# FindoraNetwork/ark-bulletproofs

Measured on AMD Instinct MI355X. Metric: r1cs_constraints_proved_per_sec (+ r1cs_batch_verifies_per_sec under "verify"), higher is better.
Workload: dtype u32x9 (256-bit modular integers, radix 2^29)

## Files before the change

### ark_bulletproofs_amd/csrc/arkbp.hip

```cpp
#include <hip/hip_runtime.h>
#include <sys/prctl.h>
#include <time.h>
#include <rccl/rccl.h>
#include <dlfcn.h>
#include <mutex>
#include <cmath>
#include <cstdio>
#include <cstring>
#include <algorithm>
#include <deque>
#include <array>
#include <functional>
#include <map>
#include <memory>
#include <set>
#include <string>
#include <tuple>
#include <unordered_map>
#include <vector>
#include "../../include/arkbp.h"
#include <atomic>
#include <chrono>
#include "host_proto.hpp"
#include "prove_steps.hpp"
// ... 780 lines not shown
    HIPCHK(ctx_stream_wait(ctx));
    HIPCHK(hipGetLastError());
    const double t_m3 = mtrace ? tnow() : 0;
    result = use_marginals ? msm_horner_tail<C>((const u64*)ctx->h_T, pl.W * pl.c, 0, 0, 1) : msm_horner_tail<C>((const u64*)ctx->h_T, 0, pl.W, nblk_ws, pl.c);
    if (mtrace) fprintf(stderr, "[msm] n=%zu c=%d W=%d K=%d  front(enqueue+sync) %.1f us  back enqueue %.1f us  back wait %.1f us  host tail %.1f us\n", n, pl.c, pl.W, K,
                        (t_m1 - t_m0) * 1e6, (t_m2 - t_m1) * 1e6, (t_m3 - t_m2) * 1e6, (tnow() - t_m3) * 1e6);
    return finish_sharded(result);
}

struct FbRun { int table; size_t first, count; size_t stride = 1; };
template <class C> static int fb_rows_build(hipStream_t st, const u32* gens, u32* table, size_t count, size_t table_cap, size_t slab, DevBuf& tmp, DevBuf& pref, DevBuf& outb) {
    for (size_t lo = 0; lo < count; lo += slab) {
        const size_t m = std::min(slab, count - lo);
        const u32 gb = (u32)((m + 255) / 256);
        hipLaunchKernelGGL(k_msm_fb_rows<C>, dim3(gb), dim3(256), 0, st, gens + lo * 16, tmp.as<u32>(), (u32)m, FB_ROWS);
        hipLaunchKernelGGL(k_ftab_normalize<C>, dim3(gb), dim3(256), 0, st, tmp.as<u32>(), pref.as<u32>(), outb.as<u32>(), (u32)m, FB_ROWS);
        HIPCHK(hipGetLastError());
        for (u32 r = 0; r < FB_ROWS; r++)
            HIPCHK(hipMemcpyAsync(table + ((size_t)r * table_cap + lo) * 16, outb.as<u32>() + (size_t)r * m * 16, m * 64, hipMemcpyDeviceToDevice, st));
    }
    return BP_OK;
}
template <class C> static int fb_tables_build(bp_ctx* ctx, size_t cap) {
    hipStream_t st = ctx->stream;
    if (cap == 0 || cap > ctx->gens_cap) { g_err = "msm tables: more bases than installed generators"; return BP_E_GENS_LENGTH; }
    if (!ctx->d_G.owned) { g_err = "msm tables: build them on the ctx that owns the generator tables, then bp_gens_share"; return BP_E_ARG; }
    ctx->fb_cap = 0;
    BPCHK(ctx->fb_G.ensure_exact((size_t)FB_ROWS * cap * 64)); BPCHK(ctx->fb_H.ensure_exact((size_t)FB_ROWS * cap * 64)); BPCHK(ctx->fb_pc.ensure((size_t)FB_ROWS * 2 * 64));
    const size_t slab = std::min<size_t>(cap, (size_t)1 << 18);
    DevBuf tmp, pref, outb;
    BPCHK(tmp.ensure(FB_ROWS * slab * 96)); BPCHK(pref.ensure(FB_ROWS * slab * 32)); BPCHK(outb.ensure(FB_ROWS * slab * 64));
// ... 360 lines not shown
    typedef host::Fld<typename C::Fr> S;
    memset(&d, 0, sizeof d);
    d.nwin = (u32)ctx->ftab_nwin;
    if (d.nwin > 44) return false;
    if constexpr (C::HAS_GLV) {
        GlvRaw raw; u32 dummy[5];
        if (!glv_decompose<C>(t, dummy, dummy, dummy, dummy, &raw)) return false;
        ftab_recode(raw.mg1, 3, raw.n1, ctx->ftab_w, ctx->ftab_nwin, d.e1, d.neg1);
        ftab_recode(raw.mg2, 3, raw.n2, ctx->ftab_w, ctx->ftab_nwin, d.e2, d.neg2);
    } else {
        uint64_t c[4]; S::to_canon(c, t);
        ftab_recode(c, 4, false, ctx->ftab_w, ctx->ftab_nwin, d.e1, d.neg1);
    }
    return true;
}
template <class C> static int ftab_build(bp_ctx* ctx, size_t n, int w, size_t budget_bytes, u32 first = 0, u32 stride = 1) {
    hipStream_t st = ctx->stream;
    if (n == 0 || stride == 0 || (size_t)first + (n - 1) * (size_t)stride >= ctx->gens_cap) { g_err = "fold tables: more bases than installed generators"; return BP_E_GENS_LENGTH; }
    if (!ctx->d_G.owned && stride == 1) { g_err = "fold tables: build them on the ctx that owns the generator tables, then bp_gens_share"; return BP_E_ARG; }
    for (DevBuf* b : {&ctx->ftab_G, &ctx->ftab_H}) { if (!b->owned) { b->p = nullptr; b->cap = 0; b->owned = true; } else b->release(); }
    ctx->ftab_n = 0; ctx->ftab_first = 0; ctx->ftab_stride = 1;
    size_t free_b = 0, total_b = 0;
    HIPCHK(hipMemGetInfo(&free_b, &total_b));
    if (!budget_bytes) budget_bytes = free_b / 4 * 3;
    auto bytes_for = [&](int ww) { const size_t E = (size_t)1 << (ww - 1); return 2 * (size_t)ftab_nwin_for<C>(ww) * E * n * 64 + E * n * (96 + 32) + n * 96; };
    if (w == 0) { w = 8; while (w > 2 && bytes_for(w) > budget_bytes) w--; }
    if (w < 2 || w > 8 || bytes_for(w) > free_b) { g_err = "fold tables: not enough device memory"; return BP_E_ARG; }
    const size_t E = (size_t)1 << (w - 1);
    const int nwin = ftab_nwin_for<C>(w);
    const size_t per_vec = (size_t)nwin * E * n * 64;
    BPCHK(ctx->ftab_G.ensure_exact(per_vec)); BPCHK(ctx->ftab_H.ensure_exact(per_vec));
    DevBuf tmp, pref, state, gsl;
    BPCHK(tmp.ensure_exact(E * n * 96)); BPCHK(pref.ensure_exact(E * n * 32)); BPCHK(state.ensure_exact(n * 96));
    const u32 gb = (u32)((n + 255) / 256);
    if (stride > 1 || first) BPCHK(gsl.ensure_exact(n * 64));
    for (int v = 0; v < 2; v++) {
        const u32* gens = v ? ctx->d_H.as<u32>() : ctx->d_G.as<u32>();
        if (gsl.p) {
            hipLaunchKernelGGL(k_cyclic_gather<Blk64>, dim3(gb), dim3(256), 0, st, gens, gsl.as<u32>(), (u32)n, first, stride);
            gens = gsl.as<u32>();
        }
        u32* T = v ? ctx->ftab_H.as<u32>() : ctx->ftab_G.as<u32>();
        for (int j = 0; j < nwin; j++) {
            hipLaunchKernelGGL(k_ftab_window<C>, dim3(gb), dim3(256), 0, st, gens, state.as<u32>(), tmp.as<u32>(), (u32)n, (u32)E, j == 0 ? 1 : 0);
            hipLaunchKernelGGL(k_ftab_normalize<C>, dim3(gb), dim3(256), 0, st, tmp.as<u32>(), pref.as<u32>(), T + (size_t)j * E * n * 16, (u32)n, (u32)E);
        }
    }
    HIPCHK(hipGetLastError());
    HIPCHK(ctx_stream_wait(ctx));
    tmp.release(); pref.release(); state.release(); gsl.release();
    ctx->ftab_n = n; ctx->ftab_w = w; ctx->ftab_nwin = nwin; ctx->ftab_first = first; ctx->ftab_stride = stride;
    return BP_OK;
}
template <class C> static int tables_check(bp_ctx* ctx, uint64_t* bad_fold, uint64_t* bad_rows) {
    hipStream_t st = ctx->stream;
    BPCHK(ctx->io_out.ensure(64));
    unsigned long long* d_bad = ctx->io_out.as<unsigned long long>();
    HIPCHK(hipMemsetAsync(d_bad, 0, 16, st));
    if (ctx->ftab_n) {
        const u32 n = (u32)ctx->ftab_n, E = 1u << (ctx->ftab_w - 1), gb = (n + 255) / 256;
// ... 137 lines not shown
    IpaState s;
    if (!ladder) {
        if (!ctx->ftab_n || !ctx->ftab_G.p || !ctx->ftab_H.p) { g_err = "bp_debug_fold: the fold tables are not built (bp_gens_fold_tables)"; return BP_E_ARG; }
        if (!stride || (size_t)first + (in_pts - 1) * (size_t)stride >= ctx->gens_cap) { g_err = "bp_debug_fold: an element lies outside the installed generators"; return BP_E_ARG; }
        s.gens_first = first; s.gens_stride = stride;
        u32 c0 = 0, cs = 1;
        const size_t tabled = tab2 ? 3 * n : n;
        if (!ftab_cols(ctx, s, c0, cs) || (size_t)c0 + (tabled - 1) * (size_t)cs >= ctx->ftab_n) { g_err = "bp_debug_fold: an element lies outside the fold tables"; return BP_E_ARG; }
    }
    DevBuf wG, wH, out;
    auto done = [&](int rc) { wG.release(); wH.release(); out.release(); return rc; };
#define DFCHK(x) do { int rc__ = (x); if (rc__ != BP_OK) return done(rc__); } while (0)
#define DFHIP(x) do { if ((x) != hipSuccess) { g_err = "bp_debug_fold: HIP error"; return done(BP_E_HIP); } } while (0)
    DFCHK(wG.ensure_exact(in_pts * 64)); DFCHK(wH.ensure_exact(in_pts * 64)); DFCHK(out.ensure_exact(2 * n * 64));
    u32 *d_G = wG.as<u32>(), *d_H = wH.as<u32>();
    if (ladder) {
        DFHIP(hipMemcpyAsync(d_G, G_xy, 2 * n * 64, hipMemcpyHostToDevice, st));
        DFHIP(hipMemcpyAsync(d_H, H_xy, 2 * n * 64, hipMemcpyHostToDevice, st));
        DFCHK(bp_points_import(ctx, d_G, d_G, 2 * n)); DFCHK(bp_points_import(ctx, d_H, d_H, 2 * n));
    } else if (whole) {
        s.d_G_in = ctx->d_G.as<u32>(); s.d_H_in = ctx->d_H.as<u32>();
    } else {
        const u32 gb = (u32)((in_pts + 255) / 256);
        hipLaunchKernelGGL(k_cyclic_gather<Blk64>, dim3(gb), dim3(256), 0, st, ctx->d_G.as<u32>(), d_G, (u32)in_pts, first, stride);
        hipLaunchKernelGGL(k_cyclic_gather<Blk64>, dim3(gb), dim3(256), 0, st, ctx->d_H.as<u32>(), d_H, (u32)in_pts, first, stride);
        s.d_G_in = d_G; s.d_H_in = d_H;
    }
    ctx->fold_took = 0;
    bool ran = true;
    if (ladder) DFCHK(launch_uniform_fold<C>(ctx, d_G, d_H, n, tG, tH, 3, route == BP_DEBUG_FOLD_LADDER_NAF));
    else if (!tab2) DFCHK(launch_tab_fold<C>(ctx, s, d_G, d_H, n, tG, tH, ran));
    else { s.def_tG = tG; s.def_tH = tH; DFCHK(launch_tab_fold2<C>(ctx, s, d_G, d_H, n, t2G, t2H, ran)); }
    DFHIP(hipGetLastError());
    *took = ran ? ctx->fold_took : 0;
    if (ran) {
        DFCHK(bp_points_export(ctx, d_G, out.p, n)); DFCHK(bp_points_export(ctx, d_H, out.as<u32>() + n * 16, n));
        DFHIP(hipMemcpyAsync(G_out, out.p, n * 64, hipMemcpyDeviceToHost, st));
        DFHIP(hipMemcpyAsync(H_out, out.as<u32>() + n * 16, n * 64, hipMemcpyDeviceToHost, st));
    }
    DFHIP(ctx_stream_wait(ctx));
#undef DFCHK
#undef DFHIP
    return done(BP_OK);
}

static inline u32 dt_base_pc(int which ) { return (u32)which; }
static inline u32 dt_base_G(const bp_ctx* ctx, size_t i) { (void)ctx; return (u32)(2 + i); }
static inline u32 dt_base_H(const bp_ctx* ctx, size_t i) { return (u32)(2 + ctx->dt_cap + i); }
template <class C> static int dt_ensure(bp_ctx* ctx, size_t N, bool& ready) {
    ready = false;
    if (!ctx->tune_direct_max || N == 0 || N > ctx->tune_direct_max || ctx->shard_world > 1 || ctx->gens_cap < N) return BP_OK;
    if (ctx->dt_cap >= N) { ready = true; return BP_OK; }
    if (!ctx->dt_tab.owned && ctx->dt_tab.p) { ctx->dt_tab.p = nullptr; ctx->dt_tab.cap = 0; ctx->dt_tab.owned = true; }
// ... 2095 lines not shown
        const bool built = t.p && size && t.cap >= size;
        *dptr = built ? t.p : nullptr; *nbytes = built ? size : 0;
        return BP_OK;
    }
    DevBuf& b = which == 0 ? c->ftab_G : which == 1 ? c->ftab_H : which == 2 ? c->fb_G : c->fb_H;
    const size_t used = which < 2 ? (c->ftab_n ? (size_t)c->ftab_nwin * ((size_t)1 << (c->ftab_w - 1)) * c->ftab_n * 64 : 0) : (size_t)FB_ROWS * c->fb_cap * 64;
    *dptr = used ? b.p : nullptr; *nbytes = used;
    return BP_OK;
}
int bp_debug_fold(bp_ctx* c, int route, size_t n, const uint64_t tG[4], const uint64_t tH[4], const uint64_t t2G[4], const uint64_t t2H[4], uint32_t gens_first,
                  uint32_t gens_stride, const uint64_t* G_xy, const uint64_t* H_xy, uint64_t* G_out_xy, uint64_t* H_out_xy, uint32_t* took) {
    if (!c || route < BP_DEBUG_FOLD_LADDER || route > BP_DEBUG_FOLD_TAB2 || !n || n >= ((size_t)1 << 28) || !tG || !tH || !G_out_xy || !H_out_xy || !took) {
        g_err = "bp_debug_fold: bad argument"; return BP_E_ARG;
    }
    if (route == BP_DEBUG_FOLD_TAB2 && (!t2G || !t2H)) { g_err = "bp_debug_fold: the second multipliers are missing"; return BP_E_ARG; }
    if (route <= BP_DEBUG_FOLD_LADDER_NAF && (!G_xy || !H_xy)) { g_err = "bp_debug_fold: the ladder routes fold the caller's points"; return BP_E_ARG; }
    if (c->host_only) return BP_E_NO_DEVICE;
    HIPCHK(hipSetDevice(c->device));
    return c->curve == 0 ? dbg_fold<Secq>(c, route, n, tG, tH, t2G, t2H, gens_first, gens_stride, G_xy, H_xy, G_out_xy, H_out_xy, took)
                         : dbg_fold<Zorro>(c, route, n, tG, tH, t2G, t2H, gens_first, gens_stride, G_xy, H_xy, G_out_xy, H_out_xy, took);
}
int bp_debug_msm_direct(bp_ctx* c, size_t njobs, const uint32_t* desc, const uint64_t* imm, const uint64_t* const* scalars, const size_t* scalar_lens,
                        uint64_t* out_xy, uint32_t* workgroups) {
    if (!c || !desc || !out_xy || njobs < 1 || njobs > (size_t)DT_MAXOUT) { g_err = "bp_debug_msm_direct: bad argument"; return BP_E_ARG; }
    if (c->host_only) return BP_E_NO_DEVICE;
    if (!c->dt_cap || !c->dt_tab.p) { g_err = "bp_debug_msm_direct: the direct tables are not built (bp_gens_direct_tables)"; return BP_E_ARG; }
    HIPCHK(hipSetDevice(c->device));
    return c->curve == 0 ? dbg_msm_direct<Secq>(c, njobs, desc, imm, scalars, scalar_lens, out_xy, workgroups)
                         : dbg_msm_direct<Zorro>(c, njobs, desc, imm, scalars, scalar_lens, out_xy, workgroups);
}
int bp_gens_download(bp_ctx* c, uint64_t* G_xy, uint64_t* H_xy, size_t n) {
// ... 817 lines not shown
```

### ark_bulletproofs_amd/csrc/ipa.cuh

```cuda
#pragma once
#include "msm.cuh"

namespace arkbp {

template <class F> __global__ void k_scalars_import(const u32* __restrict__ in, u32* __restrict__ out, u32 n) {
    const u32 i = blockIdx.x * blockDim.x + threadIdx.x;
    if (i >= n) return;
    u32 w[8];
    load_words8(w, in + (size_t)i * 8);
    store_fe_dev<F>(out + (size_t)i * 8, fe_load_ark<F>(w));
}
template <class F> __global__ void k_scalars_export(const u32* __restrict__ in, u32* __restrict__ out, u32 n) {
    const u32 i = blockIdx.x * blockDim.x + threadIdx.x;
    if (i >= n) return;
    u32 w[8];
    fe_store_ark<F>(w, load_fe_dev<F>(in + (size_t)i * 8));
    store_words8(out + (size_t)i * 8, w);
}

static constexpr int IMPORT_MAX = 5;
struct ImportList {
    u32* dst[IMPORT_MAX];
    u32 cnt[IMPORT_MAX];
    int nseg;
// ... 298 lines not shown
    if (first) {
        c1 = fe_mul<F>(c1, load_fe_dev<F>(Vf + (size_t)i * 8));
        c2 = fe_mul<F>(c2, load_fe_dev<F>(Vf + (size_t)(n + i) * 8));
    }
    u32 s1[8], s2[8];
    fe_store_canon<F>(s1, c1);
    fe_store_canon<F>(s2, c2);
    const Aff P1 = load_aff_dev(V + (size_t)i * 16), P2 = load_aff_dev(V + (size_t)(n + i) * 16);
    const Jac r = shamir2<C>(P1, P2, s1, s2);
    fold_emit<C>(V, i, t, r, jac_ws);
}

struct Naf {
    u32 plus[9], minus[9];
};
template <class C> __device__ __forceinline__ Jac ladder_madd(const Jac& acc, const Aff& T) {
    bool rare;
    Jac nxt = jac_madd_fast<C>(acc, T, rare);
    if (__builtin_expect(rare, 0)) nxt = jac_madd<C>(acc, T);
    return nxt;
}
template <class C, bool QUAD = false> __global__ void __launch_bounds__(256) __attribute__((amdgpu_waves_per_eu(2)))
k_ipa_fold_uniform(u32* __restrict__ G, u32* __restrict__ H, u32 n, Naf tG, Naf tH, int which ,
                   u32* __restrict__ jac_ws) {
    const u32 tl = blockIdx.x * blockDim.x + threadIdx.x;
    const u32 t = QUAD ? tl >> 2 : tl, ql = threadIdx.x & 3u;
    if (t >= (which == 3 ? 2 * n : n)) return;
    const bool isH = which == 2 || (which == 3 && t >= n);
    const u32 i = (which == 3 && isH) ? t - n : t;
    u32* V = isH ? H : G;
    const Aff P1 = load_aff_dev(V + (size_t)i * 16), P2 = load_aff_dev(V + (size_t)(n + i) * 16);
    const Aff N1 = aff_cneg_lazy<C>(P1, true);
    Jac acc = jac_inf<C>();
#pragma unroll 1
    for (int wd = 8; wd >= 0; wd--) {
        const u32 ep = isH ? tH.plus[wd] : tG.plus[wd], em = isH ? tH.minus[wd] : tG.minus[wd];
#pragma unroll 1
        for (int bit = (wd == 8 ? 0 : 31); bit >= 0; bit--) {
            acc = QUAD ? qjac_dbl<C>(acc, ql) : jac_dbl<C>(acc);
            if (((ep | em) >> bit) & 1) {
                Aff T1 = P1; T1.y = ((em >> bit) & 1) ? N1.y : P1.y;
                acc = QUAD ? qjac_madd<C>(acc, T1, ql) : ladder_madd<C>(acc, T1);
            }
        }
    }
    acc = QUAD ? qjac_madd<C>(acc, P2, ql) : jac_madd<C>(acc, P2);
    if (!QUAD || ql == 0) fold_emit<C>(V, i, t, acc, jac_ws);
}

struct Naf2 {
    u32 p1[5], m1[5], p2[5], m2[5];
};
template <class C, bool QUAD = false> __global__ void __launch_bounds__(256) __attribute__((amdgpu_waves_per_eu(2)))
k_ipa_fold_glv(u32* __restrict__ G, u32* __restrict__ H, u32 n, Naf2 tG, Naf2 tH, int which ,
               u32* __restrict__ jac_ws) {
    typedef typename C::Fq F;
    const u32 tl = blockIdx.x * blockDim.x + threadIdx.x;
    const u32 t = QUAD ? tl >> 2 : tl, ql = threadIdx.x & 3u;
    if (t >= (which == 3 ? 2 * n : n)) return;
    const bool isH = which == 2 || (which == 3 && t >= n);
    const u32 i = (which == 3 && isH) ? t - n : t;
    u32* V = isH ? H : G;
    const Aff P1 = load_aff_dev(V + (size_t)i * 16), P2 = load_aff_dev(V + (size_t)(n + i) * 16);
    Aff Q1;
    Q1.x = fe_canon<F>(fe_mul<F>(P1.x, fe_const<F, C::BETA29>()));
    Q1.y = P1.y;
    const Aff N1 = aff_cneg_lazy<C>(P1, true);
    Jac acc = jac_inf<C>();
#pragma unroll 1
    for (int wd = 4; wd >= 0; wd--) {
        const u32 a = isH ? tH.p1[wd] : tG.p1[wd], b = isH ? tH.m1[wd] : tG.m1[wd];
        const u32 c = isH ? tH.p2[wd] : tG.p2[wd], d = isH ? tH.m2[wd] : tG.m2[wd];
#pragma unroll 1
        for (int bit = (wd == 4 ? 1 : 31); bit >= 0; bit--) {
            acc = QUAD ? qjac_dbl<C>(acc, ql) : jac_dbl<C>(acc);
            if (QUAD) {
                if (((a | b) >> bit) & 1) { Aff T1 = P1; T1.y = ((b >> bit) & 1) ? N1.y : P1.y; acc = qjac_madd<C>(acc, T1, ql); }
                if (((c | d) >> bit) & 1) { Aff T2 = Q1; T2.y = ((d >> bit) & 1) ? N1.y : P1.y; acc = qjac_madd<C>(acc, T2, ql); }
            } else {
#pragma unroll 1
                for (int h = 0; h < 2; h++) {
                    const u32 nz = h ? (c | d) : (a | b), ng = h ? d : b;
                    if ((nz >> bit) & 1) {
                        Aff T;
#pragma unroll
                        for (int l = 0; l < 9; l++) { T.x.l[l] = h ? Q1.x.l[l] : P1.x.l[l]; T.y.l[l] = ((ng >> bit) & 1) ? N1.y.l[l] : P1.y.l[l]; }
                        acc = ladder_madd<C>(acc, T);
                    }
                }
            }
        }
    }
    acc = QUAD ? qjac_madd<C>(acc, P2, ql) : jac_madd<C>(acc, P2);
    if (!QUAD || ql == 0) fold_emit<C>(V, i, t, acc, jac_ws);
}

struct FtabDigits {
    unsigned short e1[44], e2[44];
    unsigned long long neg1, neg2;
    u32 nwin;
};
template <class C> __global__ void __launch_bounds__(256)
k_ftab_window(const u32* __restrict__ gens, u32* __restrict__ state, u32* __restrict__ tmp, u32 n, u32 E, int first) {
    const u32 i = blockIdx.x * blockDim.x + threadIdx.x;
    if (i >= n) return;
    Jac B;
    if (first) { const Aff p = load_aff_dev(gens + (size_t)i * 16); B = jac_madd<C>(jac_inf<C>(), p); }
    else B = load_jac_ws(state + (size_t)i * 24);
    Jac acc = B;
    store_jac_ws<C>(tmp + (size_t)i * 24, acc);
#pragma unroll 1
    for (u32 e = 2; e <= E; e++) {
        acc = jac_add<C>(acc, B);
        store_jac_ws<C>(tmp + ((size_t)(e - 1) * n + i) * 24, acc);
    }
    store_jac_ws<C>(state + (size_t)i * 24, jac_dbl<C>(acc));
}
template <class C> __global__ void __launch_bounds__(256)
k_ftab_normalize(const u32* __restrict__ tmp, u32* __restrict__ pref, u32* __restrict__ out, u32 n, u32 E) {
    typedef typename C::Fq F;
    const u32 i = blockIdx.x * blockDim.x + threadIdx.x;
    if (i >= n) return;
    Fe acc = fe_one<F>();
#pragma unroll 1
    for (u32 e = 0; e < E; e++) {
        u32 w[8];
        load_words8(w, tmp + ((size_t)e * n + i) * 24 + 16);
        const Fe z = fe_unpack(w);
        if (!fe_is_zero_exact(z)) acc = fe_mul<F>(acc, z);
        fe_pack(w, fe_canon<F>(acc));
        store_words8(pref + ((size_t)e * n + i) * 8, w);
    }
    Fe inv = fe_inv<F>(acc);
#pragma unroll 1
    for (int e = (int)E - 1; e >= 0; e--) {
        const Jac P = load_jac_ws(tmp + ((size_t)e * n + i) * 24);
        Aff o;
        if (jac_is_inf(P)) { o.x = fe_zero<F>(); o.y = fe_zero<F>(); }
        else {
            Fe prev = fe_one<F>();
            if (e > 0) { u32 w[8]; load_words8(w, pref + ((size_t)(e - 1) * n + i) * 8); prev = fe_unpack(w); }
            const Fe zinv = fe_mul<F>(inv, prev);
            inv = fe_mul<F>(inv, P.Z);
            o = jac_to_aff_with_zinv<C>(P, zinv);
        }
        u32 w[16];
        aff_store_dev(w, o);
        store_words8(out + ((size_t)e * n + i) * 16, w);
        store_words8(out + ((size_t)e * n + i) * 16 + 8, w + 8);
    }
}
template <class C> __device__ __forceinline__ bool jac_equals_aff(const Jac& J, const Aff& A) {
    typedef typename C::Fq F;
    const bool ji = jac_is_inf(J), ai = aff_is_inf(A);
    if (ji || ai) return ji && ai;
    const Fe zz = fe_sqr<F>(J.Z);
    if (!fe_eq_mod<F>(fe_wred<F>(J.X), fe_mul<F>(A.x, zz))) return false;
    return fe_eq_mod<F>(fe_wred<F>(J.Y), fe_mul<F>(A.y, fe_mul<F>(zz, J.Z)));
}
template <class C> __device__ __forceinline__ bool chain_entry_ok(const u32* __restrict__ cur, const u32* __restrict__ p, const u32* __restrict__ q, bool identity_ok) {
    typedef typename C::Fq F;
    bool canon, unused;
    const Aff A = load_aff_checked<C>(cur, canon);
    const Aff P = load_aff_checked<C>(p, unused);
// ... 123 lines not shown
```

### ark_bulletproofs_amd/csrc/msm.cuh

```cuda
#pragma once
#include "ec.cuh"
#include "fe_io.cuh"
#include "ecq.cuh"
#include "glv.cuh"
#include "msm_plan.hpp"

namespace arkbp {

static constexpr int MSM_MAXSEG = 6;

struct BaseSegs {
    const u32* ptr[MSM_MAXSEG];
    u32 start[MSM_MAXSEG + 1];
    int nseg;
    u32 fixed_c4;
    u32 tbits;
    u64 row_words[MSM_MAXSEG];
    u32 glv;
    u32 stride[MSM_MAXSEG];
};
__device__ __forceinline__ const u32* seg_base_ptr(const BaseSegs& s, u32 idx) {
    u32 w = 0;
    if (s.glv) idx >>= 1;
    if (s.fixed_c4) { w = idx >> s.tbits; idx &= (1u << s.tbits) - 1u; }
    const u32* ptr = s.ptr[0];
    u32 start = s.start[0], sd = s.stride[0];
    u64 rw = s.row_words[0];
#pragma unroll
    for (int j = 1; j < MSM_MAXSEG; j++) {
        const bool in = j < s.nseg && idx >= s.start[j];
        ptr = in ? s.ptr[j] : ptr; start = in ? s.start[j] : start; sd = in ? s.stride[j] : sd; rw = in ? s.row_words[j] : rw;
    }
    sd = sd ? sd : 1u;
    return ptr + (size_t)(idx - start) * sd * 16 + (size_t)(w * s.fixed_c4) * rw;
}

struct ScalSegs {
    const u32* ptr[MSM_MAXSEG];
    u32 start[MSM_MAXSEG + 1];
    int nseg;
};
__device__ __forceinline__ const u32* seg_scalar_ptr(const ScalSegs& s, u32 idx) {
    int k = 0;
#pragma unroll
    for (int j = 1; j < MSM_MAXSEG; j++) k += (j < s.nseg && idx >= s.start[j]) ? 1 : 0;
    return s.ptr[k] + (size_t)(idx - s.start[k]) * 8;
}

template <class T> struct PerJob { T j[MSM_JOBS]; };
// ... 420 lines not shown
        const bool valid = live && d != 0 && w >= pl.w_lo && w < pl.w_hi;
        const u32 pos = wave_count(cursor, (u32)w * pl.NB + (u32)(d < 0 ? -d : d) - 1, valid);
        if (valid) entries[pos] = (i << 1) | (d < 0 ? 1u : 0u);
    }
}

__device__ __forceinline__ u32 find_bucket(const u32* __restrict__ off, u32 B, u32 j) {
    u32 lo = 0, hi = B;
    while (hi - lo > 1) {
        u32 mid = (lo + hi) >> 1;
        if (off[mid] <= j) lo = mid; else hi = mid;
    }
    return lo;
}

template <class C> __global__ void __launch_bounds__(256)
k_msm_accum(BaseSegs segs, const u32* __restrict__ entries, const u32* __restrict__ off0, const u32* __restrict__ off1, u32* __restrict__ out,
            u32 B, u32 nchunks, int slotted, SlotPlan sp, u32 NB, const u32* __restrict__ boff, int chl) {
    const u32 j = blockIdx.x * blockDim.x + threadIdx.x;
    if (j >= nchunks) return;
    const u32 b = find_bucket(off1, B, j);
    u32 beg, end;
    const u32 r = j - off1[b], k = off1[b + 1] - off1[b];
    u32 s0, cnt;
    if (slotted == 2) {
        s0 = boff[b]; cnt = off0[b + 1] - off0[b];
    } else if (slotted) {
        const u32 w = b / NB, v = b - w * NB;
        s0 = sp.base[w] + v * sp.cap[w]; cnt = off0[b + 1] - off0[b];
    } else {
        s0 = off0[b]; cnt = off0[b + 1] - off0[b];
    }
    const u32 per = k > 1 ? (cnt + k - 1) / k : (1u << chl);
    beg = s0 + min(r * per, cnt);
    end = min(beg + per, s0 + cnt);
    Jac acc = jac_inf<C>();
    if (beg < end) {
        u32 ent = entries[beg];
        u32 ent_n = beg + 1 < end ? entries[beg + 1] : 0u;
        Raw16 raw = load_raw16(seg_base_ptr(segs, ent >> 1));
        for (u32 e = beg; e < end; e++) {
            Raw16 raw_n = raw;
            u32 ent_nn = 0;
            if (e + 1 < end) raw_n = load_raw16(seg_base_ptr(segs, ent_n >> 1));
            if (e + 2 < end) ent_nn = entries[e + 2];
            const Aff p = aff_from_raw(raw);
            if (e == beg) {
                acc = jac_from_aff<C>(aff_cneg_lazy<C>(p, ent & 1));
                acc.Y = fe_wred<typename C::Fq>(acc.Y);
            } else {
                bool rare;
                Jac nxt = jac_madd_fast<C>(acc, aff_cneg_lazy<C>(p, ent & 1), rare);
                if (__builtin_expect(rare, 0)) nxt = jac_madd<C>(acc, aff_cneg_lazy<C>(load_aff_dev(seg_base_ptr(segs, ent >> 1)), ent & 1));
                acc = nxt;
            }
            ent = ent_n; ent_n = ent_nn;
            raw = raw_n;
        }
    }
    store_jac_ws<C>(out + (size_t)j * 24, acc);
}

template <class C> __global__ void __launch_bounds__(256)
k_msm_accum_wave(BaseSegs segs, const u32* __restrict__ entries, const u32* __restrict__ off0, const u32* __restrict__ off_last, u32* __restrict__ out, u32 B,
                 int slotted, SlotPlan sp, u32 NB, const u32* __restrict__ boff) {
    __shared__ u32 sh[4][64 * 27];
    const u32 wv = threadIdx.x >> 6, lane = threadIdx.x & 63;
    const u32 b = blockIdx.x * 4 + wv;
    if (b >= B) return;
    const u32 cnt = off0[b + 1] - off0[b];
    if (!cnt) return;
    u32 beg;
// ... 285 lines not shown
        exclc += (cn + chm) / chcap;
    }
    if (tid == 255) bin_chunks[w * bp.NBIN + bin] = exclc;
    if (big > MSM_FS_BUCKET_MAX) *overflow = 1u;
    __syncthreads();
    for (u32 x = tid; x < n; x += 256) {
        const u32 e = buf[x];
        const u32 pos = atomicAdd(&cnt[(e >> 1) & fmask], 1u);
        ent[region + pos] = ((e >> (bp.LB + 1)) << 1) | (e & 1u);
    }
}
__device__ __forceinline__ void fs_bin_range(u32 x, const MsmPlan& pl, const BinPlan& bp, u32& b0, u32& nb) {
    if (x < bp.wb * bp.NBIN) { const u32 w = x / bp.NBIN, bin = x - w * bp.NBIN; b0 = w * (u32)pl.NB + (bin << bp.LB); nb = 1u << bp.LB; }
    else { b0 = ((u32)pl.W - 1u) * (u32)pl.NB; nb = bp.top_nb; }
}
template <class C> __global__ void __launch_bounds__(256)
k_msm_accum_fs(PerJob<BaseSegs> bjobs, const u32* __restrict__ entries, const u32* __restrict__ bcnt, const u32* __restrict__ loff, const u32* __restrict__ boff,
               const u32* __restrict__ bin_chunks, u32* __restrict__ out, MsmPlan pl, BinPlan bp, FsPlan fp, u32 chcap, u32* __restrict__ info, FsJobs jb) {
    __shared__ u32 base[MSM_FS_MAXBINS + 1];
    __shared__ u32 ws[4];
    const u32 job = blockIdx.z;
    const BaseSegs& segs = bjobs.j[job];
    entries += job * jb.slots; bcnt += job * jb.buckets; loff += job * jb.buckets; boff += job * jb.buckets; bin_chunks += job * jb.binch;
    out += job * jb.part; info += job * jb.T;
    fs_block_scan(bin_chunks, fp.nbins, base, ws);
    const u32 total = min(base[fp.nbins], fp.max_chunks);
    if (blockIdx.x == 0 && threadIdx.x == 0) { info[0] = base[fp.nbins]; info[1] = base[fp.nbins - 1]; }
    const u32 j = blockIdx.x * 256u + threadIdx.x;
    if (j >= total) return;
    u32 lo = 0, hi = fp.nbins;
    while (hi - lo > 1) { const u32 mid = (lo + hi) >> 1; if (base[mid] <= j) lo = mid; else hi = mid; }
    const u32 jj = j - base[lo];
    u32 b0, nb;
    fs_bin_range(lo, pl, bp, b0, nb);
    u32 l2 = 0, h2 = nb;
    while (h2 - l2 > 1) { const u32 mid = (l2 + h2) >> 1; if (loff[b0 + mid] <= jj) l2 = mid; else h2 = mid; }
    const u32 b = b0 + l2;
    const u32 s0 = boff[b];
    const u32 cnt = bcnt[b], r = jj - loff[b];
    const u32 k = (cnt + chcap - 1u) / chcap;
    const u32 per = k > 1 ? (cnt + k - 1) / k : chcap;
    const u32 beg = s0 + min(r * per, cnt);
    const u32 end = min(beg + per, s0 + cnt);
    Jac acc = jac_inf<C>();
    if (beg < end) {
        u32 ent = entries[beg];
        u32 ent_n = beg + 1 < end ? entries[beg + 1] : 0u;
        Raw16 raw = load_raw16(seg_base_ptr(segs, ent >> 1));
        for (u32 e = beg; e < end; e++) {
            Raw16 raw_n = raw;
            u32 ent_nn = 0;
            if (e + 1 < end) raw_n = load_raw16(seg_base_ptr(segs, ent_n >> 1));
            if (e + 2 < end) ent_nn = entries[e + 2];
            Aff p = aff_from_raw(raw);
            if constexpr (C::HAS_GLV) {
                if (segs.glv && (ent & 2u) && !aff_is_inf(p)) p.x = fe_mul<typename C::Fq>(p.x, fe_const<typename C::Fq, C::BETA29>());
            }
            if (e == beg) {
                acc = jac_from_aff<C>(aff_cneg_lazy<C>(p, ent & 1));
                acc.Y = fe_wred<typename C::Fq>(acc.Y);
            } else {
                bool rare;
                Jac nxt = jac_madd_fast<C>(acc, aff_cneg_lazy<C>(p, ent & 1), rare);
                if (__builtin_expect(rare, 0)) {
                    Aff q = load_aff_dev(seg_base_ptr(segs, ent >> 1));
                    if constexpr (C::HAS_GLV) {
                        if (segs.glv && (ent & 2u) && !aff_is_inf(q)) q.x = fe_mul<typename C::Fq>(q.x, fe_const<typename C::Fq, C::BETA29>());
                    }
                    nxt = jac_madd<C>(acc, aff_cneg_lazy<C>(q, ent & 1));
                }
                acc = nxt;
            }
            ent = ent_n; ent_n = ent_nn;
            raw = raw_n;
        }
    }
    store_jac_ws<C>(out + (size_t)j * 24, acc);
}
template <class C, bool QUAD = false> __global__ void __launch_bounds__(256)
k_msm_reduce_fs(const u32* __restrict__ part, const u32* __restrict__ bcnt, const u32* __restrict__ loff, const u32* __restrict__ bin_chunks,
                u32* __restrict__ sums, MsmPlan pl, BinPlan bp, FsPlan fp, u32 chcap, u32 G, FsJobs jb) {
    __shared__ u32 base[MSM_FS_MAXBINS + 1];
    __shared__ u32 ws[4];
    const u32 job = blockIdx.z;
    part += job * jb.part; bcnt += job * jb.buckets; loff += job * jb.buckets; bin_chunks += job * jb.binch; sums += job * jb.sums;
    fs_block_scan(bin_chunks, fp.nbins, base, ws);
    const u32 g = blockIdx.x * 256u + threadIdx.x;
    const u32 nbk = bp.wb * (u32)pl.NB;
    const u32 gb = G == 4 ? g >> 2 : g;
// ... 219 lines not shown
```

Baseline: 17.76 million.

## Restructure ladder and bucket-accumulate loops, add per-block segment tables and occupancy hints

The uniform and GLV fold ladders, and the MSM bucket-accumulate kernels, now run their rare-case full point addition outside the hot loop. The loop breaks out, does the slow add once, then resumes, so the hot path keeps fewer live registers. Fold ladders also reload the base point per digit instead of holding it, and waves-per-EU hints are set per curve. MSM accumulate kernels fill a shared-memory segment table once per block to make base-pointer lookup cheaper. Fold-table building is sliced into fixed-size scratch chunks to cap temporary memory, and the debug fold path now accepts only G or only H. The risks are extra global loads per ladder digit and a block-wide sync in the accumulate kernels.

```diff
diff --git a/ark_bulletproofs_amd/csrc/arkbp.hip b/ark_bulletproofs_amd/csrc/arkbp.hip
--- a/ark_bulletproofs_amd/csrc/arkbp.hip
+++ b/ark_bulletproofs_amd/csrc/arkbp.hip
@@ -818,7 +818,7 @@
         const size_t m = std::min(slab, count - lo);
         const u32 gb = (u32)((m + 255) / 256);
         hipLaunchKernelGGL(k_msm_fb_rows<C>, dim3(gb), dim3(256), 0, st, gens + lo * 16, tmp.as<u32>(), (u32)m, FB_ROWS);
-        hipLaunchKernelGGL(k_ftab_normalize<C>, dim3(gb), dim3(256), 0, st, tmp.as<u32>(), pref.as<u32>(), outb.as<u32>(), (u32)m, FB_ROWS);
+        hipLaunchKernelGGL(k_ftab_normalize<C>, dim3(gb), dim3(256), 0, st, tmp.as<u32>(), pref.as<u32>(), outb.as<u32>(), (u32)m, FB_ROWS, 0u, (u32)m);
         HIPCHK(hipGetLastError());
         for (u32 r = 0; r < FB_ROWS; r++)
             HIPCHK(hipMemcpyAsync(table + ((size_t)r * table_cap + lo) * 16, outb.as<u32>() + (size_t)r * m * 16, m * 64, hipMemcpyDeviceToDevice, st));
@@ -1209,6 +1209,7 @@
     }
     return true;
 }
+static constexpr size_t FTAB_SCRATCH_BYTES = (size_t)1 << 30;
 template <class C> static int ftab_build(bp_ctx* ctx, size_t n, int w, size_t budget_bytes, u32 first = 0, u32 stride = 1) {
     hipStream_t st = ctx->stream;
     if (n == 0 || stride == 0 || (size_t)first + (n - 1) * (size_t)stride >= ctx->gens_cap) { g_err = "fold tables: more bases than installed generators"; return BP_E_GENS_LENGTH; }
@@ -1218,7 +1219,13 @@
     size_t free_b = 0, total_b = 0;
     HIPCHK(hipMemGetInfo(&free_b, &total_b));
     if (!budget_bytes) budget_bytes = free_b / 4 * 3;
-    auto bytes_for = [&](int ww) { const size_t E = (size_t)1 << (ww - 1); return 2 * (size_t)ftab_nwin_for<C>(ww) * E * n * 64 + E * n * (96 + 32) + n * 96; };
+    auto slice_for = [&](int ww) {
+        const size_t E = (size_t)1 << (ww - 1);
+        size_t ns = std::max<size_t>(256, FTAB_SCRATCH_BYTES / (E * 128 + 96) / 256 * 256);
+        if (const char* v = getenv("ARKBP_FTAB_SLICE")) { const long f = atol(v); if (f > 0) ns = (size_t)f; }
+        return std::min(ns, n);
+    };
+    auto bytes_for = [&](int ww) { const size_t E = (size_t)1 << (ww - 1); return 2 * (size_t)ftab_nwin_for<C>(ww) * E * n * 64 + slice_for(ww) * (E * (96 + 32) + 96); };
     if (w == 0) { w = 8; while (w > 2 && bytes_for(w) > budget_bytes) w--; }
     if (w < 2 || w > 8 || bytes_for(w) > free_b) { g_err = "fold tables: not enough device memory"; return BP_E_ARG; }
     const size_t E = (size_t)1 << (w - 1);
@@ -1226,7 +1233,8 @@
     const size_t per_vec = (size_t)nwin * E * n * 64;
     BPCHK(ctx->ftab_G.ensure_exact(per_vec)); BPCHK(ctx->ftab_H.ensure_exact(per_vec));
     DevBuf tmp, pref, state, gsl;
-    BPCHK(tmp.ensure_exact(E * n * 96)); BPCHK(pref.ensure_exact(E * n * 32)); BPCHK(state.ensure_exact(n * 96));
+    const size_t ns = slice_for(w);
+    BPCHK(tmp.ensure_exact(E * ns * 96)); BPCHK(pref.ensure_exact(E * ns * 32)); BPCHK(state.ensure_exact(ns * 96));
     const u32 gb = (u32)((n + 255) / 256);
     if (stride > 1 || first) BPCHK(gsl.ensure_exact(n * 64));
     for (int v = 0; v < 2; v++) {
@@ -1236,9 +1244,12 @@
             gens = gsl.as<u32>();
         }
         u32* T = v ? ctx->ftab_H.as<u32>() : ctx->ftab_G.as<u32>();
-        for (int j = 0; j < nwin; j++) {
-            hipLaunchKernelGGL(k_ftab_window<C>, dim3(gb), dim3(256), 0, st, gens, state.as<u32>(), tmp.as<u32>(), (u32)n, (u32)E, j == 0 ? 1 : 0);
-            hipLaunchKernelGGL(k_ftab_normalize<C>, dim3(gb), dim3(256), 0, st, tmp.as<u32>(), pref.as<u32>(), T + (size_t)j * E * n * 16, (u32)n, (u32)E);
+        for (size_t c0 = 0; c0 < n; c0 += ns) {
+            const u32 nc = (u32)std::min(ns, n - c0), sb = (nc + 255) / 256;
+            for (int j = 0; j < nwin; j++) {
+                hipLaunchKernelGGL(k_ftab_window<C>, dim3(sb), dim3(256), 0, st, gens, state.as<u32>(), tmp.as<u32>(), nc, (u32)E, j == 0 ? 1 : 0, (u32)c0);
+                hipLaunchKernelGGL(k_ftab_normalize<C>, dim3(sb), dim3(256), 0, st, tmp.as<u32>(), pref.as<u32>(), T + (size_t)j * E * n * 16, nc, (u32)E, (u32)c0, (u32)n);
+            }
         }
     }
     HIPCHK(hipGetLastError());
@@ -1406,10 +1417,10 @@
 #define DFHIP(x) do { if ((x) != hipSuccess) { g_err = "bp_debug_fold: HIP error"; return done(BP_E_HIP); } } while (0)
     DFCHK(wG.ensure_exact(in_pts * 64)); DFCHK(wH.ensure_exact(in_pts * 64)); DFCHK(out.ensure_exact(2 * n * 64));
     u32 *d_G = wG.as<u32>(), *d_H = wH.as<u32>();
+    const int which = ladder ? (G_xy ? 1 : 0) | (H_xy ? 2 : 0) : 3;
     if (ladder) {
-        DFHIP(hipMemcpyAsync(d_G, G_xy, 2 * n * 64, hipMemcpyHostToDevice, st));
-        DFHIP(hipMemcpyAsync(d_H, H_xy, 2 * n * 64, hipMemcpyHostToDevice, st));
-        DFCHK(bp_points_import(ctx, d_G, d_G, 2 * n)); DFCHK(bp_points_import(ctx, d_H, d_H, 2 * n));
+        if (G_xy) { DFHIP(hipMemcpyAsync(d_G, G_xy, 2 * n * 64, hipMemcpyHostToDevice, st)); DFCHK(bp_points_import(ctx, d_G, d_G, 2 * n)); }
+        if (H_xy) { DFHIP(hipMemcpyAsync(d_H, H_xy, 2 * n * 64, hipMemcpyHostToDevice, st)); DFCHK(bp_points_import(ctx, d_H, d_H, 2 * n)); }
     } else if (whole) {
         s.d_G_in = ctx->d_G.as<u32>(); s.d_H_in = ctx->d_H.as<u32>();
     } else {
@@ -1420,15 +1431,14 @@
     }
     ctx->fold_took = 0;
     bool ran = true;
-    if (ladder) DFCHK(launch_uniform_fold<C>(ctx, d_G, d_H, n, tG, tH, 3, route == BP_DEBUG_FOLD_LADDER_NAF));
+    if (ladder) DFCHK(launch_uniform_fold<C>(ctx, d_G, d_H, n, tG, tH, which, route == BP_DEBUG_FOLD_LADDER_NAF));
     else if (!tab2) DFCHK(launch_tab_fold<C>(ctx, s, d_G, d_H, n, tG, tH, ran));
     else { s.def_tG = tG; s.def_tH = tH; DFCHK(launch_tab_fold2<C>(ctx, s, d_G, d_H, n, t2G, t2H, ran)); }
     DFHIP(hipGetLastError());
     *took = ran ? ctx->fold_took : 0;
     if (ran) {
-        DFCHK(bp_points_export(ctx, d_G, out.p, n)); DFCHK(bp_points_export(ctx, d_H, out.as<u32>() + n * 16, n));
-        DFHIP(hipMemcpyAsync(G_out, out.p, n * 64, hipMemcpyDeviceToHost, st));
-        DFHIP(hipMemcpyAsync(H_out, out.as<u32>() + n * 16, n * 64, hipMemcpyDeviceToHost, st));
+        if (which & 1) { DFCHK(bp_points_export(ctx, d_G, out.p, n)); DFHIP(hipMemcpyAsync(G_out, out.p, n * 64, hipMemcpyDeviceToHost, st)); }
+        if (which & 2) { DFCHK(bp_points_export(ctx, d_H, out.as<u32>() + n * 16, n)); DFHIP(hipMemcpyAsync(H_out, out.as<u32>() + n * 16, n * 64, hipMemcpyDeviceToHost, st)); }
     }
     DFHIP(ctx_stream_wait(ctx));
 #undef DFCHK
@@ -3554,7 +3564,7 @@
         g_err = "bp_debug_fold: bad argument"; return BP_E_ARG;
     }
     if (route == BP_DEBUG_FOLD_TAB2 && (!t2G || !t2H)) { g_err = "bp_debug_fold: the second multipliers are missing"; return BP_E_ARG; }
-    if (route <= BP_DEBUG_FOLD_LADDER_NAF && (!G_xy || !H_xy)) { g_err = "bp_debug_fold: the ladder routes fold the caller's points"; return BP_E_ARG; }
+    if (route <= BP_DEBUG_FOLD_LADDER_NAF && !G_xy && !H_xy) { g_err = "bp_debug_fold: the ladder routes fold the caller's points"; return BP_E_ARG; }
     if (c->host_only) return BP_E_NO_DEVICE;
     HIPCHK(hipSetDevice(c->device));
     return c->curve == 0 ? dbg_fold<Secq>(c, route, n, tG, tH, t2G, t2H, gens_first, gens_stride, G_xy, H_xy, G_out_xy, H_out_xy, took)
diff --git a/ark_bulletproofs_amd/csrc/ipa.cuh b/ark_bulletproofs_amd/csrc/ipa.cuh
--- a/ark_bulletproofs_amd/csrc/ipa.cuh
+++ b/ark_bulletproofs_amd/csrc/ipa.cuh
@@ -336,13 +336,17 @@
 struct Naf {
     u32 plus[9], minus[9];
 };
-template <class C> __device__ __forceinline__ Jac ladder_madd(const Jac& acc, const Aff& T) {
-    bool rare;
-    Jac nxt = jac_madd_fast<C>(acc, T, rare);
-    if (__builtin_expect(rare, 0)) nxt = jac_madd<C>(acc, T);
-    return nxt;
-}
-template <class C, bool QUAD = false> __global__ void __launch_bounds__(256) __attribute__((amdgpu_waves_per_eu(2)))
+template <class C> struct LadderWaves { static constexpr int N = 3; };
+template <> struct LadderWaves<Zorro> { static constexpr int N = 2; };
+template <class C> __device__ __forceinline__ Aff ladder_digit(const u32* __restrict__ src, bool phi, bool neg) {
+    typedef typename C::Fq F;
+    asm volatile("" ::: "memory");
+    const Aff P1 = load_aff_dev(src);
+    Aff T = aff_cneg_lazy<C>(P1, neg);
+    if constexpr (C::HAS_GLV) { if (phi && !aff_is_inf(P1)) T.x = fe_mul<F>(P1.x, fe_const<F, C::BETA29>()); }
+    return T;
+}
+template <class C, bool QUAD = false> __global__ void __launch_bounds__(256) __attribute__((amdgpu_waves_per_eu(QUAD ? 2 : LadderWaves<C>::N)))
 k_ipa_fold_uniform(u32* __restrict__ G, u32* __restrict__ H, u32 n, Naf tG, Naf tH, int which ,
                    u32* __restrict__ jac_ws) {
     const u32 tl = blockIdx.x * blockDim.x + threadIdx.x;
@@ -351,29 +355,62 @@
     const bool isH = which == 2 || (which == 3 && t >= n);
     const u32 i = (which == 3 && isH) ? t - n : t;
     u32* V = isH ? H : G;
-    const Aff P1 = load_aff_dev(V + (size_t)i * 16), P2 = load_aff_dev(V + (size_t)(n + i) * 16);
-    const Aff N1 = aff_cneg_lazy<C>(P1, true);
-    Jac acc = jac_inf<C>();
-#pragma unroll 1
-    for (int wd = 8; wd >= 0; wd--) {
-        const u32 ep = isH ? tH.plus[wd] : tG.plus[wd], em = isH ? tH.minus[wd] : tG.minus[wd];
-#pragma unroll 1
-        for (int bit = (wd == 8 ? 0 : 31); bit >= 0; bit--) {
-            acc = QUAD ? qjac_dbl<C>(acc, ql) : jac_dbl<C>(acc);
-            if (((ep | em) >> bit) & 1) {
-                Aff T1 = P1; T1.y = ((em >> bit) & 1) ? N1.y : P1.y;
-                acc = QUAD ? qjac_madd<C>(acc, T1, ql) : ladder_madd<C>(acc, T1);
-            }
-        }
-    }
-    acc = QUAD ? qjac_madd<C>(acc, P2, ql) : jac_madd<C>(acc, P2);
-    if (!QUAD || ql == 0) fold_emit<C>(V, i, t, acc, jac_ws);
+    if constexpr (QUAD) {
+        const Aff P1 = load_aff_dev(V + (size_t)i * 16), P2 = load_aff_dev(V + (size_t)(n + i) * 16);
+        const Aff N1 = aff_cneg_lazy<C>(P1, true);
+        Jac acc = jac_inf<C>();
+#pragma unroll 1
+        for (int wd = 8; wd >= 0; wd--) {
+            const u32 ep = isH ? tH.plus[wd] : tG.plus[wd], em = isH ? tH.minus[wd] : tG.minus[wd];
+#pragma unroll 1
+            for (int bit = (wd == 8 ? 0 : 31); bit >= 0; bit--) {
+                acc = qjac_dbl<C>(acc, ql);
+                if (((ep | em) >> bit) & 1) {
+                    Aff T1 = P1; T1.y = ((em >> bit) & 1) ? N1.y : P1.y;
+                    acc = qjac_madd<C>(acc, T1, ql);
+                }
+            }
+        }
+        acc = qjac_madd<C>(acc, P2, ql);
+        if (ql == 0) fold_emit<C>(V, i, t, acc, jac_ws);
+    } else {
+        const u32* P1 = V + (size_t)i * 16;
+        const Naf& tn = isH ? tH : tG;
+        Jac acc = jac_inf<C>();
+        bool started = false;
+        int pos = 256;
+        while (pos >= 0) {
+            bool redo = false, neg = false;
+#pragma unroll 1
+            for (; pos >= 0; pos--) {
+                const u32 ep = tn.plus[pos >> 5] >> (pos & 31), em = tn.minus[pos >> 5] >> (pos & 31);
+                if (started) acc = jac_dbl<C>(acc);
+                if ((ep | em) & 1) {
+                    neg = em & 1;
+                    const Aff T = ladder_digit<C>(P1, false, neg);
+                    if (!started) {
+                        acc = jac_from_aff<C>(T);
+                        acc.Y = fe_wred<typename C::Fq>(acc.Y);
+                        started = true;
+                    } else {
+                        bool rare;
+                        const Jac nxt = jac_madd_fast<C>(acc, T, rare);
+                        if (__builtin_expect(rare, 0)) { redo = true; break; }
+                        acc = nxt;
+                    }
+                }
+            }
+            if (redo) { acc = jac_madd<C>(acc, ladder_digit<C>(P1, false, neg)); pos--; }
+        }
+        acc = jac_madd<C>(acc, load_aff_dev(V + (size_t)(n + i) * 16));
+        fold_emit<C>(V, i, t, acc, jac_ws);
+    }
 }
 
 struct Naf2 {
     u32 p1[5], m1[5], p2[5], m2[5];
 };
-template <class C, bool QUAD = false> __global__ void __launch_bounds__(256) __attribute__((amdgpu_waves_per_eu(2)))
+template <class C, bool QUAD = false> __global__ void __launch_bounds__(256) __attribute__((amdgpu_waves_per_eu(QUAD ? 2 : LadderWaves<C>::N)))
 k_ipa_fold_glv(u32* __restrict__ G, u32* __restrict__ H, u32 n, Naf2 tG, Naf2 tH, int which ,
                u32* __restrict__ jac_ws) {
     typedef typename C::Fq F;
@@ -383,38 +420,60 @@
     const bool isH = which == 2 || (which == 3 && t >= n);
     const u32 i = (which == 3 && isH) ? t - n : t;
     u32* V = isH ? H : G;
-    const Aff P1 = load_aff_dev(V + (size_t)i * 16), P2 = load_aff_dev(V + (size_t)(n + i) * 16);
-    Aff Q1;
-    Q1.x = fe_canon<F>(fe_mul<F>(P1.x, fe_const<F, C::BETA29>()));
-    Q1.y = P1.y;
-    const Aff N1 = aff_cneg_lazy<C>(P1, true);
-    Jac acc = jac_inf<C>();
-#pragma unroll 1
-    for (int wd = 4; wd >= 0; wd--) {
-        const u32 a = isH ? tH.p1[wd] : tG.p1[wd], b = isH ? tH.m1[wd] : tG.m1[wd];
-        const u32 c = isH ? tH.p2[wd] : tG.p2[wd], d = isH ? tH.m2[wd] : tG.m2[wd];
-#pragma unroll 1
-        for (int bit = (wd == 4 ? 1 : 31); bit >= 0; bit--) {
-            acc = QUAD ? qjac_dbl<C>(acc, ql) : jac_dbl<C>(acc);
-            if (QUAD) {
+    if constexpr (QUAD) {
+        const Aff P1 = load_aff_dev(V + (size_t)i * 16), P2 = load_aff_dev(V + (size_t)(n + i) * 16);
+        Aff Q1;
+        Q1.x = fe_canon<F>(fe_mul<F>(P1.x, fe_const<F, C::BETA29>()));
+        Q1.y = P1.y;
+        const Aff N1 = aff_cneg_lazy<C>(P1, true);
+        Jac acc = jac_inf<C>();
+#pragma unroll 1
+        for (int wd = 4; wd >= 0; wd--) {
+            const u32 a = isH ? tH.p1[wd] : tG.p1[wd], b = isH ? tH.m1[wd] : tG.m1[wd];
+            const u32 c = isH ? tH.p2[wd] : tG.p2[wd], d = isH ? tH.m2[wd] : tG.m2[wd];
+#pragma unroll 1
+            for (int bit = (wd == 4 ? 1 : 31); bit >= 0; bit--) {
+                acc = qjac_dbl<C>(acc, ql);
                 if (((a | b) >> bit) & 1) { Aff T1 = P1; T1.y = ((b >> bit) & 1) ? N1.y : P1.y; acc = qjac_madd<C>(acc, T1, ql); }
                 if (((c | d) >> bit) & 1) { Aff T2 = Q1; T2.y = ((d >> bit) & 1) ? N1.y : P1.y; acc = qjac_madd<C>(acc, T2, ql); }
-            } else {
-#pragma unroll 1
-                for (int h = 0; h < 2; h++) {
-                    const u32 nz = h ? (c | d) : (a | b), ng = h ? d : b;
-                    if ((nz >> bit) & 1) {
-                        Aff T;
-#pragma unroll
-                        for (int l = 0; l < 9; l++) { T.x.l[l] = h ? Q1.x.l[l] : P1.x.l[l]; T.y.l[l] = ((ng >> bit) & 1) ? N1.y.l[l] : P1.y.l[l]; }
-                        acc = ladder_madd<C>(acc, T);
+            }
+        }
+        acc = qjac_madd<C>(acc, P2, ql);
+        if (ql == 0) fold_emit<C>(V, i, t, acc, jac_ws);
+    } else {
+        const u32* P1 = V + (size_t)i * 16;
+        const Naf2& tn = isH ? tH : tG;
+        Jac acc = jac_inf<C>();
+        bool started = false;
+        int s = 259;
+        while (s >= 0) {
+            bool redo = false, neg = false, phi = false;
+#pragma unroll 1
+            for (; s >= 0; s--) {
+                const int bit = s >> 1;
+                phi = !(s & 1);
+                if (!phi && started) acc = jac_dbl<C>(acc);
+                const u32 ep = (phi ? tn.p2[bit >> 5] : tn.p1[bit >> 5]) >> (bit & 31), em = (phi ? tn.m2[bit >> 5] : tn.m1[bit >> 5]) >> (bit & 31);
+                if ((ep | em) & 1) {
+                    neg = em & 1;
+                    const Aff T = ladder_digit<C>(P1, phi, neg);
+                    if (!started) {
+                        acc = jac_from_aff<C>(T);
+                        acc.Y = fe_wred<F>(acc.Y);
+                        started = true;
+                    } else {
+                        bool rare;
+                        const Jac nxt = jac_madd_fast<C>(acc, T, rare);
+                        if (__builtin_expect(rare, 0)) { redo = true; break; }
+                        acc = nxt;
                     }
                 }
             }
-        }
-    }
-    acc = QUAD ? qjac_madd<C>(acc, P2, ql) : jac_madd<C>(acc, P2);
-    if (!QUAD || ql == 0) fold_emit<C>(V, i, t, acc, jac_ws);
+            if (redo) { acc = jac_madd<C>(acc, ladder_digit<C>(P1, phi, neg)); s--; }
+        }
+        acc = jac_madd<C>(acc, load_aff_dev(V + (size_t)(n + i) * 16));
+        fold_emit<C>(V, i, t, acc, jac_ws);
+    }
 }
 
 struct FtabDigits {
@@ -423,11 +482,11 @@
     u32 nwin;
 };
 template <class C> __global__ void __launch_bounds__(256)
-k_ftab_window(const u32* __restrict__ gens, u32* __restrict__ state, u32* __restrict__ tmp, u32 n, u32 E, int first) {
+k_ftab_window(const u32* __restrict__ gens, u32* __restrict__ state, u32* __restrict__ tmp, u32 n, u32 E, int first, u32 col0) {
     const u32 i = blockIdx.x * blockDim.x + threadIdx.x;
     if (i >= n) return;
     Jac B;
-    if (first) { const Aff p = load_aff_dev(gens + (size_t)i * 16); B = jac_madd<C>(jac_inf<C>(), p); }
+    if (first) { const Aff p = load_aff_dev(gens + (size_t)(col0 + i) * 16); B = jac_madd<C>(jac_inf<C>(), p); }
     else B = load_jac_ws(state + (size_t)i * 24);
     Jac acc = B;
     store_jac_ws<C>(tmp + (size_t)i * 24, acc);
@@ -439,7 +498,7 @@
     store_jac_ws<C>(state + (size_t)i * 24, jac_dbl<C>(acc));
 }
 template <class C> __global__ void __launch_bounds__(256)
-k_ftab_normalize(const u32* __restrict__ tmp, u32* __restrict__ pref, u32* __restrict__ out, u32 n, u32 E) {
+k_ftab_normalize(const u32* __restrict__ tmp, u32* __restrict__ pref, u32* __restrict__ out, u32 n, u32 E, u32 col0, u32 n_row) {
     typedef typename C::Fq F;
     const u32 i = blockIdx.x * blockDim.x + threadIdx.x;
     if (i >= n) return;
@@ -468,8 +527,8 @@
         }
         u32 w[16];
         aff_store_dev(w, o);
-        store_words8(out + ((size_t)e * n + i) * 16, w);
-        store_words8(out + ((size_t)e * n + i) * 16 + 8, w + 8);
+        store_words8(out + ((size_t)e * n_row + col0 + i) * 16, w);
+        store_words8(out + ((size_t)e * n_row + col0 + i) * 16 + 8, w + 8);
     }
 }
 template <class C> __device__ __forceinline__ bool jac_equals_aff(const Jac& J, const Aff& A) {
diff --git a/ark_bulletproofs_amd/csrc/msm.cuh b/ark_bulletproofs_amd/csrc/msm.cuh
--- a/ark_bulletproofs_amd/csrc/msm.cuh
+++ b/ark_bulletproofs_amd/csrc/msm.cuh
@@ -33,6 +33,31 @@
     }
     sd = sd ? sd : 1u;
     return ptr + (size_t)(idx - start) * sd * 16 + (size_t)(w * s.fixed_c4) * rw;
+}
+
+struct SegTab { uint4 a[MSM_MAXSEG]; uint2 rw[MSM_MAXSEG]; };
+__device__ __forceinline__ void seg_tab_fill(SegTab& t, const BaseSegs& s) {
+    if (threadIdx.x == 0) {
+#pragma unroll
+        for (int j = 0; j < MSM_MAXSEG; j++) {
+            const u64 p = (u64)(uintptr_t)s.ptr[j];
+            t.a[j] = make_uint4((u32)p, (u32)(p >> 32), s.stride[j] ? s.stride[j] : 1u, s.start[j]);
+            t.rw[j] = make_uint2((u32)s.row_words[j], (u32)(s.row_words[j] >> 32));
+        }
+    }
+    __syncthreads();
+}
+__device__ __forceinline__ const u32* seg_base_ptr(const BaseSegs& s, const SegTab& t, u32 idx) {
+    u32 w = 0;
+    if (s.glv) idx >>= 1;
+    if (s.fixed_c4) { w = idx >> s.tbits; idx &= (1u << s.tbits) - 1u; }
+    u32 k = 0;
+#pragma unroll
+    for (int j = 1; j < MSM_MAXSEG; j++) k += (j < s.nseg && idx >= s.start[j]) ? 1u : 0u;
+    const uint4 a = t.a[k];
+    const u32* ptr = (const u32*)(uintptr_t)(((u64)a.y << 32) | a.x) + (size_t)(idx - a.w) * a.z * 16;
+    if (s.fixed_c4) { const uint2 r = t.rw[k]; ptr += (size_t)(w * s.fixed_c4) * (((u64)r.y << 32) | r.x); }
+    return ptr;
 }
 
 struct ScalSegs {
@@ -483,9 +508,13 @@
     return lo;
 }
 
-template <class C> __global__ void __launch_bounds__(256)
+template <class C> struct AccumWaves { static constexpr int N = 2; };
+template <> struct AccumWaves<Secq> { static constexpr int N = 3; };
+template <class C> __global__ void __launch_bounds__(256) __attribute__((amdgpu_waves_per_eu(AccumWaves<C>::N)))
 k_msm_accum(BaseSegs segs, const u32* __restrict__ entries, const u32* __restrict__ off0, const u32* __restrict__ off1, u32* __restrict__ out,
             u32 B, u32 nchunks, int slotted, SlotPlan sp, u32 NB, const u32* __restrict__ boff, int chl) {
+    __shared__ SegTab segtab;
+    seg_tab_fill(segtab, segs);
     const u32 j = blockIdx.x * blockDim.x + threadIdx.x;
     if (j >= nchunks) return;
     const u32 b = find_bucket(off1, B, j);
@@ -507,24 +536,37 @@
     if (beg < end) {
         u32 ent = entries[beg];
         u32 ent_n = beg + 1 < end ? entries[beg + 1] : 0u;
-        Raw16 raw = load_raw16(seg_base_ptr(segs, ent >> 1));
-        for (u32 e = beg; e < end; e++) {
-            Raw16 raw_n = raw;
-            u32 ent_nn = 0;
-            if (e + 1 < end) raw_n = load_raw16(seg_base_ptr(segs, ent_n >> 1));
-            if (e + 2 < end) ent_nn = entries[e + 2];
-            const Aff p = aff_from_raw(raw);
-            if (e == beg) {
-                acc = jac_from_aff<C>(aff_cneg_lazy<C>(p, ent & 1));
-                acc.Y = fe_wred<typename C::Fq>(acc.Y);
-            } else {
-                bool rare;
-                Jac nxt = jac_madd_fast<C>(acc, aff_cneg_lazy<C>(p, ent & 1), rare);
-                if (__builtin_expect(rare, 0)) nxt = jac_madd<C>(acc, aff_cneg_lazy<C>(load_aff_dev(seg_base_ptr(segs, ent >> 1)), ent & 1));
-                acc = nxt;
+        Raw16 raw = load_raw16(seg_base_ptr(segs, segtab, ent >> 1));
+        u32 e = beg;
+        while (e < end) {
+            Raw16 raw_n;
+            u32 ent_nn;
+            bool redo = false;
+#pragma unroll 1
+            for (; e < end; e++) {
+                raw_n = raw;
+                ent_nn = 0;
+                if (e + 1 < end) raw_n = load_raw16(seg_base_ptr(segs, segtab, ent_n >> 1));
+                if (e + 2 < end) ent_nn = entries[e + 2];
+                const Aff p = aff_from_raw(raw);
+                if (e == beg) {
+                    acc = jac_from_aff<C>(aff_cneg_lazy<C>(p, ent & 1));
+                    acc.Y = fe_wred<typename C::Fq>(acc.Y);
+                } else {
+                    bool rare;
+                    const Jac nxt = jac_madd_fast<C>(acc, aff_cneg_lazy<C>(p, ent & 1), rare);
+                    if (__builtin_expect(rare, 0)) { redo = true; break; }
+                    acc = nxt;
+                }
+                ent = ent_n; ent_n = ent_nn;
+                raw = raw_n;
             }
-            ent = ent_n; ent_n = ent_nn;
-            raw = raw_n;
+            if (redo) {
+                acc = jac_madd<C>(acc, aff_cneg_lazy<C>(load_aff_dev(seg_base_ptr(segs, segtab, ent >> 1)), ent & 1));
+                ent = ent_n; ent_n = ent_nn;
+                raw = raw_n;
+                e++;
+            }
         }
     }
     store_jac_ws<C>(out + (size_t)j * 24, acc);
@@ -840,15 +882,17 @@
     if (x < bp.wb * bp.NBIN) { const u32 w = x / bp.NBIN, bin = x - w * bp.NBIN; b0 = w * (u32)pl.NB + (bin << bp.LB); nb = 1u << bp.LB; }
     else { b0 = ((u32)pl.W - 1u) * (u32)pl.NB; nb = bp.top_nb; }
 }
-template <class C> __global__ void __launch_bounds__(256)
+template <class C> __global__ void __launch_bounds__(256) __attribute__((amdgpu_waves_per_eu(AccumWaves<C>::N)))
 k_msm_accum_fs(PerJob<BaseSegs> bjobs, const u32* __restrict__ entries, const u32* __restrict__ bcnt, const u32* __restrict__ loff, const u32* __restrict__ boff,
                const u32* __restrict__ bin_chunks, u32* __restrict__ out, MsmPlan pl, BinPlan bp, FsPlan fp, u32 chcap, u32* __restrict__ info, FsJobs jb) {
     __shared__ u32 base[MSM_FS_MAXBINS + 1];
     __shared__ u32 ws[4];
+    __shared__ SegTab segtab;
     const u32 job = blockIdx.z;
     const BaseSegs& segs = bjobs.j[job];
     entries += job * jb.slots; bcnt += job * jb.buckets; loff += job * jb.buckets; boff += job * jb.buckets; bin_chunks += job * jb.binch;
     out += job * jb.part; info += job * jb.T;
+    seg_tab_fill(segtab, segs);
     fs_block_scan(bin_chunks, fp.nbins, base, ws);
     const u32 total = min(base[fp.nbins], fp.max_chunks);
     if (blockIdx.x == 0 && threadIdx.x == 0) { info[0] = base[fp.nbins]; info[1] = base[fp.nbins - 1]; }
@@ -872,33 +916,44 @@
     if (beg < end) {
         u32 ent = entries[beg];
         u32 ent_n = beg + 1 < end ? entries[beg + 1] : 0u;
-        Raw16 raw = load_raw16(seg_base_ptr(segs, ent >> 1));
-        for (u32 e = beg; e < end; e++) {
-            Raw16 raw_n = raw;
-            u32 ent_nn = 0;
-            if (e + 1 < end) raw_n = load_raw16(seg_base_ptr(segs, ent_n >> 1));
-            if (e + 2 < end) ent_nn = entries[e + 2];
-            Aff p = aff_from_raw(raw);
-            if constexpr (C::HAS_GLV) {
-                if (segs.glv && (ent & 2u) && !aff_is_inf(p)) p.x = fe_mul<typename C::Fq>(p.x, fe_const<typename C::Fq, C::BETA29>());
+        Raw16 raw = load_raw16(seg_base_ptr(segs, segtab, ent >> 1));
+        u32 e = beg;
+        while (e < end) {
+            Raw16 raw_n;
+            u32 ent_nn;
+            bool redo = false;
+#pragma unroll 1
+            for (; e < end; e++) {
+                raw_n = raw;
+                ent_nn = 0;
+                if (e + 1 < end) raw_n = load_raw16(seg_base_ptr(segs, segtab, ent_n >> 1));
+                if (e + 2 < end) ent_nn = entries[e + 2];
+                Aff p = aff_from_raw(raw);
+                if constexpr (C::HAS_GLV) {
+                    if (segs.glv && (ent & 2u) && !aff_is_inf(p)) p.x = fe_mul<typename C::Fq>(p.x, fe_const<typename C::Fq, C::BETA29>());
+                }
+                if (e == beg) {
+                    acc = jac_from_aff<C>(aff_cneg_lazy<C>(p, ent & 1));
+                    acc.Y = fe_wred<typename C::Fq>(acc.Y);
+                } else {
+                    bool rare;
+                    const Jac nxt = jac_madd_fast<C>(acc, aff_cneg_lazy<C>(p, ent & 1), rare);
+                    if (__builtin_expect(rare, 0)) { redo = true; break; }
+                    acc = nxt;
+                }
+                ent = ent_n; ent_n = ent_nn;
+                raw = raw_n;
             }
-            if (e == beg) {
-                acc = jac_from_aff<C>(aff_cneg_lazy<C>(p, ent & 1));
-                acc.Y = fe_wred<typename C::Fq>(acc.Y);
-            } else {
-                bool rare;
-                Jac nxt = jac_madd_fast<C>(acc, aff_cneg_lazy<C>(p, ent & 1), rare);
-                if (__builtin_expect(rare, 0)) {
-                    Aff q = load_aff_dev(seg_base_ptr(segs, ent >> 1));
-                    if constexpr (C::HAS_GLV) {
-                        if (segs.glv && (ent & 2u) && !aff_is_inf(q)) q.x = fe_mul<typename C::Fq>(q.x, fe_const<typename C::Fq, C::BETA29>());
-                    }
-                    nxt = jac_madd<C>(acc, aff_cneg_lazy<C>(q, ent & 1));
+            if (redo) {
+                Aff q = load_aff_dev(seg_base_ptr(segs, segtab, ent >> 1));
+                if constexpr (C::HAS_GLV) {
+                    if (segs.glv && (ent & 2u) && !aff_is_inf(q)) q.x = fe_mul<typename C::Fq>(q.x, fe_const<typename C::Fq, C::BETA29>());
                 }
-                acc = nxt;
+                acc = jac_madd<C>(acc, aff_cneg_lazy<C>(q, ent & 1));
+                ent = ent_n; ent_n = ent_nn;
+                raw = raw_n;
+                e++;
             }
-            ent = ent_n; ent_n = ent_nn;
-            raw = raw_n;
         }
     }
     store_jac_ws<C>(out + (size_t)j * 24, acc);
```

After: 17.38 million. 2.1% lower.
